# ultralytics/yolov5

Measured on NVIDIA H100. Metric: images/sec @640 (forward + NMS), higher is better.
Workload: dtype bf16

## Files before the change

yolov5_b200/csrc/conv_gemm.cu:

```cuda
#include <cstdio>
#include <cstdlib>
#include <cstring>
#include <mutex>

#include "../../include/y5b200.h"
#include "common.cuh"
#include "host_util.h"
#include "wgmma.cuh"

namespace y5 {

constexpr int kBlockM = 128;
constexpr int kConsumers = 2;
constexpr int kConsumerThreads = 128 * kConsumers;
constexpr int kThreads = 128 + kConsumerThreads;
constexpr int kMaxStages = 8;
constexpr int kHeadN = 128;

enum AMode { A_LINEAR = 0, A_IM2COL = 1, A_PATCH = 2 };

struct ConvParams {
    int M, N;
    int num_m_tiles;
    int num_m_super, num_n_tiles;
    int kh, kw, c_chunks;
    int block_k;
    int a_mode;
    int Ho, Wo, HoWo, stride, pad_h, pad_w;
    int tw, th, tiles_x, tiles_y;
    int b_grouped;
    int patch_pw;
    int cluster_n;
    uint32_t stg_bytes;
    uint32_t b_sub_bytes;
    float rcp_per_img, rcp_tiles_x, rcp_HoWo, rcp_Wo;
    int a_stages, b_stages;
    uint32_t a_sub_bytes, a_stage_bytes, b_stage_bytes;
    int is_bf16, act;
    const float* bias;
    int bias_n;
    void* out;
    int out_pitch;
    const void* res;
    int res_pitch;
    void* raw;
    void* z;
    int na, no, nc, nx, z_rows, z_row0;
    float det_stride;
    float anchor_wh[8];
};

struct SmemLayout {
    uint32_t off_a, off_b, off_out, off_bias, off_bars, total;
};

__host__ __device__ inline SmemLayout smem_layout(int epi, int no, int bias_n, int a_stages, int b_stages, uint32_t a_bytes,
                                                   uint32_t b_bytes, uint32_t stg_bytes) {
    SmemLayout L;
    uint32_t o = 0;
    L.off_a = o;
    o += a_stages * a_bytes;
    L.off_b = o;
    o += b_stages * b_bytes;
    o = (o + 1023) & ~1023u;
    L.off_out = o;
    if (epi == 1) o += 4 * ((kBlockM * no * 2 + 1023) & ~1023u);
    else o += stg_bytes;
    L.off_bias = o;
    o += ((bias_n + 3) & ~3) * 4;
    o = (o + 7) & ~7u;
    L.off_bars = o;
    o += 4 * kMaxStages * 8;
    L.total = o;
    return L;
}

__device__ __forceinline__ int fdiv(int n, int d, float rd) {
    if (n >= (1 << 23)) return n / d;
    int q = __float2int_rz(__int2float_rz(n) * rd);
    const int r = n - q * d;
    if (r >= d) ++q;
    else if (r < 0) --q;
    return q;
}

template <int BLOCK_N, int MT, int KS, bool BF16>
__device__ __forceinline__ void mma_batch(float (&acc)[MT][BLOCK_N / 2], uint32_t a_lo, uint32_t a_sub16, uint32_t a_hi, uint32_t b_lo,
                                          uint32_t b_hi, uint32_t scale_first) {
    wgmma_fence();
#pragma unroll
    for (int k = 0; k < KS; ++k)
#pragma unroll
        for (int mi = 0; mi < MT; ++mi)
            Wgmma<BLOCK_N>::template run<BF16, 0, 0>(acc[mi], gmma_desc(a_lo + mi * a_sub16 + 2 * k, a_hi), gmma_desc(b_lo + 2 * k, b_hi),
                                                     k == 0 ? scale_first : 1u);
    wgmma_commit();
}

template <int BLOCK_N, int EPI, int MT, bool OPT, bool BF16>
__global__ void __launch_bounds__(kThreads, 1)
conv_gemm_kernel(const __grid_constant__ CUtensorMap tmA, const __grid_constant__ CUtensorMap tmB, const ConvParams p) {
    static_assert(MT * BLOCK_N <= 256, "accumulators: at most 128 fp32 registers per consumer thread");
    constexpr int kAcc = BLOCK_N / 2;

    extern __shared__ __align__(1024) uint8_t smem_raw[];
    uint8_t* smem = reinterpret_cast<uint8_t*>((reinterpret_cast<uintptr_t>(smem_raw) + 1023) & ~uintptr_t(1023));
    const SmemLayout L = smem_layout(EPI, p.no, p.bias_n, p.a_stages, p.b_stages, p.a_stage_bytes, p.b_stage_bytes, p.stg_bytes);
    uint8_t* sA = smem + L.off_a;
    uint8_t* sB = smem + L.off_b;
    float* sBias = reinterpret_cast<float*>(smem + L.off_bias);
    uint64_t* a_full = reinterpret_cast<uint64_t*>(smem + L.off_bars);
    uint64_t* a_empty = a_full + kMaxStages;
    uint64_t* b_full = a_empty + kMaxStages;
    uint64_t* b_empty = b_full + kMaxStages;

    const int warp = threadIdx.x >> 5;
    const int lane = threadIdx.x & 31;
    const int csize = OPT ? static_cast<int>(cluster_nctarank()) : 1;
    const uint32_t crank = OPT ? cluster_ctarank() : 0u;

    if (threadIdx.x == 0) {
        tma_prefetch_desc(&tmA);
        tma_prefetch_desc(&tmB);
        for (int s = 0; s < kMaxStages; ++s) {
            mbar_init(&a_full[s], 1);
            mbar_init(&a_empty[s], kConsumers);
            mbar_init(&b_full[s], 1);
            mbar_init(&b_empty[s], kConsumers * csize);
        }
        fence_barrier_init();
    }
    if (threadIdx.x >= 128)
        for (int i = threadIdx.x - 128; i < p.bias_n; i += kConsumerThreads) {
            const float b = i < p.N ? __ldg(p.bias + i) : 0.0f;
            sBias[i] = (EPI == 0 && p.act) ? 0.5f * b : b;
        }
    __syncthreads();
    if (csize > 1) cluster_sync_all();
    griddep_wait();
    griddep_launch_dependents();

    const int nn = p.num_n_tiles;
    const int num_tiles = ((p.num_m_super + csize - 1) / csize) * nn;
    const int tile0 = blockIdx.x / csize, tile_step = gridDim.x / csize;
    const uint32_t row_bytes = p.block_k * 2;
    const bool patch = p.a_mode == A_PATCH;
    const bool wide = OPT && p.patch_pw > 0;
    const int grp = wide ? p.kh * p.kw : (patch ? p.kh : 1);
    const int num_groups = wide ? p.c_chunks : (patch ? p.c_chunks * p.kw : p.kh * p.kw * p.c_chunks);

    if (warp < 4) {
        setmaxnreg_dec<56>();
    }
    if (warp == 0) {
        int as = 0, bs = 0;
        uint32_t aph = 0, bph = 0;
        for (int tile = tile0; tile < num_tiles; tile += tile_step) {
            const int ms = (tile / nn) * csize + static_cast<int>(crank);
            const int n0 = (tile - (tile / nn) * nn) * BLOCK_N;
            int img[MT], y0[MT], x0[MT];
#pragma unroll
            for (int mi = 0; mi < MT; ++mi) {
                const int mt = ms * MT + mi;
                img[mi] = y0[mi] = x0[mi] = 0;
                if (p.a_mode == A_IM2COL) {
                    const int m0 = mt * kBlockM;
                    img[mi] = fdiv(m0, p.HoWo, p.rcp_HoWo);
                    const int rem = m0 - img[mi] * p.HoWo;
                    const int oy = fdiv(rem, p.Wo, p.rcp_Wo);
                    y0[mi] = oy * p.stride - p.pad_h;
                    x0[mi] = (rem - oy * p.Wo) * p.stride - p.pad_w;
                } else if (patch) {
                    const int per_img = p.tiles_x * p.tiles_y;
                    img[mi] = fdiv(mt, per_img, p.rcp_per_img);
                    const int rem = mt - img[mi] * per_img;
                    const int ty = fdiv(rem, p.tiles_x, p.rcp_tiles_x);
                    y0[mi] = ty * p.th - p.pad_h;
                    x0[mi] = (rem - ty * p.tiles_x) * p.tw - p.pad_w;
                }
            }
            auto issue_group = [&](int cc, int s, int r0) {
                mbar_wait(&a_empty[as], aph ^ 1);
                if (elect_one()) {
                    mbar_arrive_expect_tx(&a_full[as], p.a_stage_bytes);
#pragma unroll
                    for (int mi = 0; mi < MT; ++mi) {
                        uint8_t* a_dst = sA + as * p.a_stage_bytes + mi * p.a_sub_bytes;
                        if (wide) {
                            if (mi == 0) tma_load_4d(&tmA, &a_full[as], a_dst, cc * p.block_k, x0[0], y0[0], img[0]);
                        } else if (p.a_mode == A_LINEAR) tma_load_2d(&tmA, &a_full[as], a_dst, cc * p.block_k, (ms * MT + mi) * kBlockM);
                        else if (p.a_mode == A_IM2COL)
                            tma_load_im2col_4d(&tmA, &a_full[as], a_dst, cc * p.block_k, x0[mi], y0[mi], img[mi], static_cast<uint16_t>(s),
                                               static_cast<uint16_t>(r0));
                        else tma_load_4d(&tmA, &a_full[as], a_dst, cc * p.block_k, x0[mi] + s, y0[mi], img[mi]);
                    }
                }
                __syncwarp();
                if (++as == p.a_stages) { as = 0; aph ^= 1; }
// ... 10 lines not shown
                            const int slice_rows = BLOCK_N / csize;
                            tma_load_2d_mcast(&tmB, &b_full[bs], b_dst + crank * slice_rows * row_bytes, kb * p.block_k,
                                              n0 + static_cast<int>(crank) * slice_rows, static_cast<uint16_t>((1u << csize) - 1u));
                        }
                    }
                    __syncwarp();
                    if (stage_last && ++bs == p.b_stages) { bs = 0; bph ^= 1; }
                }
            };
            if (wide) {
                for (int cc = 0; cc < p.c_chunks; ++cc) issue_group(cc, 0, 0);
            } else if (patch) {
                for (int cc = 0; cc < p.c_chunks; ++cc)
                    for (int s = 0; s < p.kw; ++s) issue_group(cc, s, 0);
            } else {
                for (int r = 0; r < p.kh; ++r)
                    for (int s = 0; s < p.kw; ++s)
                        for (int cc = 0; cc < p.c_chunks; ++cc) issue_group(cc, s, r);
            }
        }
    } else if (warp >= 4) {
    setmaxnreg_inc<224>();
    const int wg = (warp >> 2) - 1;
    const int ct = threadIdx.x - 128;
    const int wrow = wg * 64 + (warp & 3) * 16 + (lane >> 2);
    const int ccol = 2 * (lane & 3);
    const bool signal = (threadIdx.x & 127) == 0;
    constexpr bool bf16 = BF16;
    const uint32_t dhi = gmma_desc_hi(row_bytes);
    const uint32_t a_hi = wide ? (dhi & ~0x3FFFu) | (((static_cast<uint32_t>(p.patch_pw) * row_bytes) >> 4) & 0x3FFFu) : dhi;
    const uint32_t a_base = gmma_desc_lo(smem_u32(sA) + (wide ? wg * 8 * p.patch_pw : wg * 64) * row_bytes), b_base = gmma_desc_lo(smem_u32(sB));
    const uint32_t row16 = row_bytes >> 4;
    const uint32_t a_stage16 = p.a_stage_bytes >> 4, b_stage16 = p.b_stage_bytes >> 4, a_sub16 = p.a_sub_bytes >> 4;
    const uint32_t b_sub16 = p.b_sub_bytes >> 4;
    const uint32_t a_shift16 = patch ? (p.tw * row_bytes) >> 4 : 0;
    const int k_steps = p.block_k / 16;
    const int per_img = p.tiles_x * p.tiles_y;
    const int tw_shift = patch ? __ffs(p.tw) - 1 : 0;
    int as = 0, bs = 0, head_set = 0;
    uint32_t aph = 0, bph = 0;
    float acc[MT][kAcc];
#pragma unroll
    for (int mi = 0; mi < MT; ++mi)
#pragma unroll
        for (int i = 0; i < kAcc; ++i) acc[mi][i] = 0.0f;

    int pend_as = 0, pend_bs = 0;
    bool pend_a_last = false, pend_b_last = false;
    auto release_pending = [&]() {
        if (!signal) return;
        if (pend_b_last) {
            if (csize == 1) mbar_arrive(&b_empty[pend_bs]);
            else
                for (int r = 0; r < csize; ++r) mbar_arrive_cluster(mapa_u32(&b_empty[pend_bs], static_cast<uint32_t>(r)));
        }
        if (pend_a_last) mbar_arrive(&a_empty[pend_as]);
    };

    for (int tile = tile0; tile < num_tiles; tile += tile_step) {
        const int ms = (tile / nn) * csize + static_cast<int>(crank);
        const int nt = tile - (tile / nn) * nn;
        const int n0 = nt * BLOCK_N;
        for (int g = 0; g < num_groups; ++g) {
            mbar_wait(&a_full[as], aph);
            const uint32_t a_stage_lo = a_base + as * a_stage16;
            uint32_t a_lo = a_stage_lo;
            for (int j = 0; j < grp; ++j) {
                if (wide) {
                    const int tr = j / p.kw, ts = j - tr * p.kw;
                    a_lo = a_stage_lo + (tr * p.patch_pw + ts) * row16;
                }
                const bool stage_first = !p.b_grouped || j == 0, stage_last = !p.b_grouped || j == grp - 1;
                if (stage_first) mbar_wait(&b_full[bs], bph);
                const uint32_t b_lo = b_base + bs * b_stage16 + (p.b_grouped ? j * b_sub16 : 0u);
                const uint32_t scale_first = (g | j) != 0 ? 1u : 0u;
#pragma unroll
                for (int mi = 0; mi < MT; ++mi) fence_regs(acc[mi]);
                switch (k_steps) {
                    case 4: mma_batch<BLOCK_N, MT, 4, BF16>(acc, a_lo, a_sub16, a_hi, b_lo, dhi, scale_first); break;
                    case 2: mma_batch<BLOCK_N, MT, 2, BF16>(acc, a_lo, a_sub16, a_hi, b_lo, dhi, scale_first); break;
                    default: mma_batch<BLOCK_N, MT, 1, BF16>(acc, a_lo, a_sub16, a_hi, b_lo, dhi, scale_first); break;
                }
                wgmma_wait<1>();
#pragma unroll
                for (int mi = 0; mi < MT; ++mi) fence_regs(acc[mi]);
                if (g | j) release_pending();
                pend_as = as;
                pend_a_last = j == grp - 1;
                pend_bs = bs;
                pend_b_last = stage_last;
                if (stage_last && ++bs == p.b_stages) { bs = 0; bph ^= 1; }
                a_lo += a_shift16;
            }
            if (++as == p.a_stages) { as = 0; aph ^= 1; }
        }
        wgmma_wait<0>();
#pragma unroll
        for (int mi = 0; mi < MT; ++mi) fence_regs(acc[mi]);
        release_pending();

        if (EPI == 0) {
            const bool staged = OPT && p.stg_bytes != 0;
            const uint32_t stg_pitch = BLOCK_N * 2 + 16;
            uint8_t* stg = smem + L.off_out + wg * 64 * stg_pitch;
            auto pixel_of = [&](int mt, int row) -> long long {
                if (patch) {
                    const int img = fdiv(mt, per_img, p.rcp_per_img);
                    const int rem = mt - img * per_img;
                    const int tyi = fdiv(rem, p.tiles_x, p.rcp_tiles_x);
                    const int oy = tyi * p.th + (row >> tw_shift), ox = (rem - tyi * p.tiles_x) * p.tw + (row & ((1 << tw_shift) - 1));
                    return (mt < p.num_m_tiles && oy < p.Ho && ox < p.Wo) ? static_cast<long long>(img) * p.HoWo + oy * p.Wo + ox : -1;
                }
                const long long m = static_cast<long long>(mt) * kBlockM + row;
                return m < p.M ? m : -1;
            };
            constexpr int kRows = 2 * MT, kWords = (OPT ? 128 : 256) / BLOCK_N;
            constexpr int kBatch = kWords < 1 ? 1 : (kWords < kRows ? kWords : kRows);
            const bool has_res = p.res != nullptr;
#pragma unroll
            for (int q0 = 0; q0 < kRows; q0 += kBatch) {
                uint32_t rv[kBatch][BLOCK_N / 8];
                long long gp[kBatch];
#pragma unroll
                for (int q = 0; q < kBatch; ++q) gp[q] = pixel_of(ms * MT + (q0 + q) / 2, wrow + 8 * ((q0 + q) & 1));
                if (has_res) {
#pragma unroll
                    for (int q = 0; q < kBatch; ++q) {
                        const uint16_t* rp = reinterpret_cast<const uint16_t*>(p.res) + (gp[q] < 0 ? 0 : gp[q] * p.res_pitch) + n0 + ccol;
#pragma unroll
                        for (int j = 0; j < BLOCK_N / 8; ++j)
                            rv[q][j] = (gp[q] >= 0 && n0 + 8 * j < p.N) ? *reinterpret_cast<const uint32_t*>(rp + 8 * j) : 0u;
                    }
                }
#pragma unroll
                for (int q = 0; q < kBatch; ++q) {
                    const int mi = (q0 + q) / 2, h = (q0 + q) & 1;
                    const int mt = ms * MT + mi;
                    const int row = wrow + 8 * h;
                    const long long gpix = gp[q];
                    if (gpix >= 0 || staged) {
                        uint16_t* op = reinterpret_cast<uint16_t*>(p.out) + gpix * p.out_pitch + n0 + ccol;
                        uint8_t* sp = stg + (row - wg * 64) * stg_pitch + ccol * 2;
#pragma unroll
                        for (int j = 0; j < BLOCK_N / 8; ++j) {
                            if (n0 + 8 * j >= p.N) continue;
                            const float2 b = *reinterpret_cast<const float2*>(sBias + n0 + 8 * j + ccol);
                            const float a0 = acc[mi][4 * j + 2 * h], a1 = acc[mi][4 * j + 2 * h + 1];
                            float f0, f1;
                            if (p.act) {
                                f0 = silu_from_half(fmaf(a0, 0.5f, b.x));
                                f1 = silu_from_half(fmaf(a1, 0.5f, b.y));
                            } else {
                                f0 = a0 + b.x;
                                f1 = a1 + b.y;
                            }
                            if (has_res && gpix >= 0) {
                                const float2 t = unpack2(rv[q][j], bf16);
                                f0 += t.x;
                                f1 += t.y;
                            }
                            if (staged) *reinterpret_cast<uint32_t*>(sp + 16 * j) = pack2(f0, f1, bf16);
                            else *reinterpret_cast<uint32_t*>(op + 8 * j) = pack2(f0, f1, bf16);
                        }
                    }
                    if (staged && h == 1) {
                        named_bar_sync(2 + wg, 128);
                        constexpr int kSeg = BLOCK_N / 8;
                        for (int i = threadIdx.x & 127; i < 64 * kSeg; i += 128) {
                            const int lrow = i / kSeg, c = i - lrow * kSeg;
                            const long long gp = pixel_of(mt, wg * 64 + lrow);
                            if (gp >= 0 && n0 + 8 * c < p.N)
                                *reinterpret_cast<uint4*>(reinterpret_cast<uint16_t*>(p.out) + gp * p.out_pitch + n0 + 8 * c) =
                                    *reinterpret_cast<const uint4*>(stg + lrow * stg_pitch + c * 16);
                        }
                        named_bar_sync(2 + wg, 128);
                    }
                }
            }
        } else {
            const uint32_t blk = (kBlockM * p.no * 2 + 1023) & ~1023u;
            const int set = head_set;
            head_set ^= 1;
            uint16_t* stage_raw = reinterpret_cast<uint16_t*>(smem + L.off_out + (2 * set) * blk);
            uint16_t* stage_z = reinterpret_cast<uint16_t*>(smem + L.off_out + (2 * set + 1) * blk);
            const int no = p.no;
            const int a = nt;
            const float aw = p.anchor_wh[a * 2], ah = p.anchor_wh[a * 2 + 1];
            const int m0 = ms * kBlockM;
            const int rows_here = min(kBlockM, p.M - m0);
#pragma unroll
            for (int h = 0; h < 2; ++h) {
                const int row = wrow + 8 * h;
                const int m = m0 + row;
                int gx = 0, gy = 0;
                if (m < p.M) { const int pix = m - fdiv(m, p.HoWo, p.rcp_HoWo) * p.HoWo; gy = fdiv(pix, p.nx, p.rcp_Wo); gx = pix - gy * p.nx; }
                const float fgx = static_cast<float>(gx) - 0.5f, fgy = static_cast<float>(gy) - 0.5f;
#pragma unroll
                for (int j = 0; j < BLOCK_N / 8; ++j) {
#pragma unroll
                    for (int e = 0; e < 2; ++e) {
                        const int o = 8 * j + ccol + e;
                        if (o >= no) continue;
                        const float x = acc[0][4 * j + 2 * h + e] + sBias[n0 + o];
                        float d = x;
                        if (o < 5 + p.nc) {
                            const float sg = sigmoid_f(x);
                            if (o == 0) d = (sg * 2.0f + fgx) * p.det_stride;
                            else if (o == 1) d = (sg * 2.0f + fgy) * p.det_stride;
                            else if (o == 2) { const float u = sg * 2.0f; d = u * u * aw; }
                            else if (o == 3) { const float u = sg * 2.0f; d = u * u * ah; }
                            else d = sg;
                        }
                        stage_raw[row * no + o] = pack1(x, bf16);
                        stage_z[row * no + o] = pack1(d, bf16);
                    }
                }
            }
            named_bar_sync(1, kConsumerThreads);
            const int b_lo = fdiv(m0, p.HoWo, p.rcp_HoWo), b_hi = fdiv(m0 + rows_here - 1, p.HoWo, p.rcp_HoWo);
            for (int b = b_lo; b <= b_hi; ++b) {
                const int r_lo = max(b * p.HoWo - m0, 0), r_hi = min((b + 1) * p.HoWo - m0, rows_here);
                const int pix_lo = m0 + r_lo - b * p.HoWo;
                const int n_el = (r_hi - r_lo) * no;
#pragma unroll
                for (int which = 0; which < 2; ++which) {
                    const long long dst_el = which == 0
                        ? ((static_cast<long long>(b) * p.na + a) * p.HoWo + pix_lo) * no
                        : (static_cast<long long>(b) * p.z_rows + p.z_row0 + static_cast<long long>(a) * p.HoWo + pix_lo) * no;
                    uint16_t* dst = reinterpret_cast<uint16_t*>(which == 0 ? p.raw : p.z) + dst_el;
                    const uint16_t* src = (which == 0 ? stage_raw : stage_z) + r_lo * no;
                    if ((((reinterpret_cast<uintptr_t>(dst) | reinterpret_cast<uintptr_t>(src)) & 15) == 0) && (n_el & 7) == 0) {
                        const uint4* s4 = reinterpret_cast<const uint4*>(src);
                        uint4* d4 = reinterpret_cast<uint4*>(dst);
                        for (int i = ct; i < n_el / 8; i += kConsumerThreads) d4[i] = s4[i];
                    } else {
                        for (int i = ct; i < n_el; i += kConsumerThreads) dst[i] = src[i];
                    }
                }
            }
        }
    }
    }
    if (csize > 1) cluster_sync_all();
}

__global__ void conv_direct_kernel(const uint16_t* __restrict__ in, long long xs, long long ys, long long ns, int B, int H,
                                   int W, int Cin, const uint16_t* __restrict__ w, int cin_pad, const float* __restrict__ bias,
                                   uint16_t* out, int out_pitch, int Cout, const uint16_t* res, int res_pitch, int kh, int kw,
                                   int stride, int pad_h, int pad_w, int Ho, int Wo, int act, int bf16) {
    const long long idx = static_cast<long long>(blockIdx.x) * blockDim.x + threadIdx.x;
    const long long total = static_cast<long long>(B) * Ho * Wo * Cout;
    if (idx >= total) return;
    const int n = static_cast<int>(idx % Cout);
    const long long m = idx / Cout;
    const int ox = static_cast<int>(m % Wo);
    const int oy = static_cast<int>((m / Wo) % Ho);
    const int b = static_cast<int>(m / (static_cast<long long>(Wo) * Ho));
    float acc = 0.0f;
    for (int r = 0; r < kh; ++r) {
        const int iy = oy * stride - pad_h + r;
        if (iy < 0 || iy >= H) continue;
        for (int s = 0; s < kw; ++s) {
            const int ix = ox * stride - pad_w + s;
            if (ix < 0 || ix >= W) continue;
            const uint16_t* ip = in + b * ns + iy * ys + ix * xs;
            const uint16_t* wp = w + (static_cast<long long>(n) * kh * kw + r * kw + s) * cin_pad;
            for (int c = 0; c < Cin; ++c) acc += unpack1(ip[c], bf16) * unpack1(wp[c], bf16);
        }
    }
    float x = acc + bias[n];
    if (act) x = x / (1.0f + expf(-x));
    if (res) x += unpack1(res[m * res_pitch + n], bf16);
    out[m * out_pitch + n] = pack1(x, bf16);
}

}

using namespace y5;

namespace {

int pick_block_k(int in_c) {
    return in_c > 16 ? 64 : 16;
}

void pick_tile(int out_c, int64_t m_tiles, int* block_n, int* mt) {
    const int64_t sms = sm_count();
    if (out_c <= 32) { *block_n = 32; *mt = 4; return; }
    if (out_c <= 64) { *block_n = 64; *mt = 2; return; }
    if (out_c <= 128) {
        *block_n = 128;
        *mt = ((m_tiles + 1) / 2) >= sms ? 2 : 1;
        return;
    }
    const int64_t tiles256 = m_tiles * ((out_c + 255) / 256);
    *block_n = (tiles256 >= 2 * sms && (out_c % 256 == 0 || out_c > 384)) ? 256 : 128;
    *mt = 1;
}

int pick_block_n(int out_c, int64_t m_rows) {
    int bn, mt;
    pick_tile(out_c, m_rows > 0 ? (m_rows + kBlockM - 1) / kBlockM : 1, &bn, &mt);
    return bn;
}

template <int BN, int EPI, int MT, bool OPT>
cudaError_t launch_conv(const CUtensorMap& a, const CUtensorMap& b, const ConvParams& p, int grid, int cluster, uint32_t smem,
                        cudaStream_t st) {
    auto* kernel = p.is_bf16 ? conv_gemm_kernel<BN, EPI, MT, OPT, true> : conv_gemm_kernel<BN, EPI, MT, OPT, false>;
    const cudaError_t attr_err = ensure_dyn_smem(reinterpret_cast<const void*>(kernel), 227 * 1024);
    if (attr_err != cudaSuccess) return attr_err;
    count_launch();
    if (cluster == 1) return launch_pdl(kernel, dim3(grid), dim3(kThreads), smem, st, a, b, p);
    static const bool pdl = [] { const char* e = getenv("Y5_PDL"); return !(e && e[0] == '0'); }();
    cudaLaunchConfig_t cfg{};
    cfg.gridDim = dim3(grid);
    cfg.blockDim = dim3(kThreads);
    cfg.dynamicSmemBytes = smem;
    cfg.stream = st;
    cudaLaunchAttribute attr[2];
    attr[0].id = cudaLaunchAttributeClusterDimension;
    attr[0].val.clusterDim.x = cluster;
    attr[0].val.clusterDim.y = 1;
    attr[0].val.clusterDim.z = 1;
    attr[1].id = cudaLaunchAttributeProgrammaticStreamSerialization;
    attr[1].val.programmaticStreamSerializationAllowed = 1;
// ... 13 lines not shown
    ConvParams& p = pc.p;
    p.cluster_n = cluster;
    p.a_stage_bytes = mt * p.a_sub_bytes;
    if (p.patch_pw > 0) p.a_stage_bytes = static_cast<uint32_t>(p.th + p.kh - 1) * p.patch_pw * p.block_k * 2;
    p.num_m_super = (p.num_m_tiles + mt - 1) / mt;
    p.num_n_tiles = epi == 1 ? p.na : (p.N + block_n - 1) / block_n;
    p.bias_n = p.num_n_tiles * block_n;
    const uint32_t budget = 225 * 1024 - 1024;
    const bool patch = p.a_mode == A_PATCH;
    int a_st = 0, b_st = 0;
    if (!patch) {
        for (int s = kMaxStages; s >= 2; --s)
            if (smem_layout(epi, p.no, p.bias_n, s, s, p.a_stage_bytes, p.b_stage_bytes, p.stg_bytes).total <= budget) { a_st = b_st = s; break; }
    } else {
        const int b_min = p.b_grouped ? 2 : 3, b_max = p.b_grouped ? 4 : kMaxStages;
        for (int a = 3; a >= 2 && !a_st; --a)
            for (int b = b_max; b >= b_min; --b)
                if (smem_layout(epi, p.no, p.bias_n, a, b, p.a_stage_bytes, p.b_stage_bytes, p.stg_bytes).total <= budget) { a_st = a; b_st = b; break; }
    }
    if (a_st < 2 || b_st < 2) return set_error(Y5_E_UNSUPPORTED, "conv tile does not fit shared memory (block_n %d a %u b %u)", block_n,
                                                p.a_stage_bytes, p.b_stage_bytes);
    p.a_stages = a_st;
    p.b_stages = b_st;
    pc.smem_bytes = smem_layout(epi, p.no, p.bias_n, a_st, b_st, p.a_stage_bytes, p.b_stage_bytes, p.stg_bytes).total + 1024;
    pc.block_n = block_n;
    pc.epi = epi;
    pc.mt = mt;
    pc.cluster = cluster;
    const long long tiles = static_cast<long long>((p.num_m_super + cluster - 1) / cluster) * p.num_n_tiles;
    const int max_clusters = sm_count() / cluster;
    pc.grid = static_cast<int>(tiles < max_clusters ? tiles : max_clusters) * cluster;
    return 0;
}

int run_plan(const PlanCommon& pc, cudaStream_t st) {
    cudaError_t e = cudaErrorInvalidValue;
    const bool opt = pc.cluster > 1 || pc.p.patch_pw > 0 || pc.p.stg_bytes > 0;
    const int key = (opt ? 100000 : 0) + pc.epi * 10000 + pc.block_n * 10 + pc.mt;
    switch (key) {
        case 324: e = launch_conv<32, 0, 4, false>(pc.tmA, pc.tmB, pc.p, pc.grid, pc.cluster, pc.smem_bytes, st); break;
        case 642: e = launch_conv<64, 0, 2, false>(pc.tmA, pc.tmB, pc.p, pc.grid, pc.cluster, pc.smem_bytes, st); break;
        case 1281: e = launch_conv<128, 0, 1, false>(pc.tmA, pc.tmB, pc.p, pc.grid, pc.cluster, pc.smem_bytes, st); break;
        case 1282: e = launch_conv<128, 0, 2, false>(pc.tmA, pc.tmB, pc.p, pc.grid, pc.cluster, pc.smem_bytes, st); break;
        case 2561: e = launch_conv<256, 0, 1, false>(pc.tmA, pc.tmB, pc.p, pc.grid, pc.cluster, pc.smem_bytes, st); break;
        case 11281: e = launch_conv<kHeadN, 1, 1, false>(pc.tmA, pc.tmB, pc.p, pc.grid, pc.cluster, pc.smem_bytes, st); break;
        case 100324: e = launch_conv<32, 0, 4, true>(pc.tmA, pc.tmB, pc.p, pc.grid, pc.cluster, pc.smem_bytes, st); break;
        case 100642: e = launch_conv<64, 0, 2, true>(pc.tmA, pc.tmB, pc.p, pc.grid, pc.cluster, pc.smem_bytes, st); break;
        case 101281: e = launch_conv<128, 0, 1, true>(pc.tmA, pc.tmB, pc.p, pc.grid, pc.cluster, pc.smem_bytes, st); break;
        case 101282: e = launch_conv<128, 0, 2, true>(pc.tmA, pc.tmB, pc.p, pc.grid, pc.cluster, pc.smem_bytes, st); break;
        case 102561: e = launch_conv<256, 0, 1, true>(pc.tmA, pc.tmB, pc.p, pc.grid, pc.cluster, pc.smem_bytes, st); break;
        default: return set_error(Y5_E_UNSUPPORTED, "conv: no kernel for block_n %d mt %d epi %d", pc.block_n, pc.mt, pc.epi);
    }
    if (e != cudaSuccess) return set_error(int(e), "conv_gemm launch failed: %s", cudaGetErrorString(e));
    return 0;
}

bool aligned16(const void* p) { return (reinterpret_cast<uintptr_t>(p) & 15) == 0; }

struct Geo {
    int kh, kw, pad_h, pad_w, Ho, Wo;
    long long xs, ys, ns;
};
Geo geometry(const y5_conv_desc* d) {
    Geo g;
    g.kh = d->ksize;
    g.kw = d->kw ? d->kw : d->ksize;
    g.pad_h = d->pad;
    g.pad_w = d->kw ? d->pad_w : d->pad;
    g.xs = d->in_x_stride ? d->in_x_stride : d->in_pitch;
    g.ys = d->in_y_stride ? d->in_y_stride : static_cast<long long>(d->in_w) * g.xs;
    g.ns = d->in_n_stride ? d->in_n_stride : static_cast<long long>(d->in_h) * g.ys;
    g.Ho = (d->in_h + 2 * g.pad_h - g.kh) / d->stride + 1;
    g.Wo = (d->in_w + 2 * g.pad_w - g.kw) / d->stride + 1;
    return g;
}

}

struct y5_conv_plan {
    PlanCommon pc;
};
struct y5_detect_plan {
    PlanCommon pc;
};

extern "C" Y5_API int y5_conv_pick(int32_t in_c, int32_t out_c, int64_t m_rows, int32_t* block_k, int32_t* block_n) {
    if (in_c <= 0 || out_c <= 0) return set_error(Y5_E_INVALID, "y5_conv_pick: non-positive channel count");
    if (block_k) *block_k = pick_block_k(in_c);
    if (block_n) *block_n = pick_block_n(out_c, m_rows);
    return 0;
}

static int validate_conv(const y5_conv_desc* d) {
    if (!d || !d->in || !d->weight || !d->bias || !d->out) return set_error(Y5_E_INVALID, "conv: null pointer");
    if (d->dtype != Y5_F16 && d->dtype != Y5_BF16) return set_error(Y5_E_UNSUPPORTED, "conv: dtype must be fp16/bf16");
    if (d->batch <= 0 || d->in_h <= 0 || d->in_w <= 0 || d->in_c <= 0 || d->out_c <= 0)
        return set_error(Y5_E_INVALID, "conv: non-positive dimension");
    const long long xs = d->in_x_stride ? d->in_x_stride : d->in_pitch;
    if (xs <= 0 || xs % 8 || (d->in_y_stride % 8) || (d->in_n_stride % 8) || d->out_pitch < d->out_c || d->out_pitch % 8 || d->out_c % 8)
        return set_error(Y5_E_INVALID, "conv: strides/pitches/out_c must be multiples of 8 elements and cover the view");
    if (!d->in_x_stride && d->in_pitch < d->in_c) return set_error(Y5_E_INVALID, "conv: in_pitch smaller than in_c");
    if (!aligned16(d->in) || !aligned16(d->out) || !aligned16(d->weight) || (d->residual && !aligned16(d->residual)))
        return set_error(Y5_E_INVALID, "conv: pointers must be 16-byte aligned");
    if (d->residual && (d->res_pitch < d->out_c || d->res_pitch % 8)) return set_error(Y5_E_INVALID, "conv: bad residual pitch");
    const int kw = d->kw ? d->kw : d->ksize, pw = d->kw ? d->pad_w : d->pad;
    if (d->ksize < 1 || d->ksize > 7 || kw < 1 || kw > 7 || d->stride < 1 || d->stride > 8 || d->pad < 0 || d->pad > d->ksize || pw < 0 ||
        pw > kw)
        return set_error(Y5_E_UNSUPPORTED, "conv: kernel %dx%d stride %d pad %d,%d unsupported", d->ksize, kw, d->stride, d->pad, pw);
    return 0;
}

extern "C" Y5_API int y5_conv_plan_create(const y5_conv_desc* d, y5_conv_plan** out) {
// ... 6 lines not shown
    if (M64 > 0x7fffffff - 256) return set_error(Y5_E_UNSUPPORTED, "conv: more than 2^31 output pixels");
    const int bk = d->block_k ? d->block_k : pick_block_k(d->in_c);
    if (bk != 16 && bk != 32 && bk != 64) return set_error(Y5_E_INVALID, "conv: block_k must be 16/32/64");
    const bool plain = g.kh == 1 && g.kw == 1 && d->stride == 1 && g.pad_h == 0 && g.pad_w == 0 && !d->in_x_stride && !d->in_y_stride &&
                       !d->in_n_stride;
    int best_tw = 0;
    double best_eff = 0.0;
    if (d->stride == 1 && !plain) {
        for (int tw = 8; tw <= 128; tw <<= 1) {
            const int th = 128 / tw;
            const double eff = (double)g.Wo * g.Ho / ((double)((g.Wo + tw - 1) / tw * tw) * ((g.Ho + th - 1) / th * th));
            if (eff > best_eff + 1e-9) { best_eff = eff; best_tw = tw; }
        }
    }
    int a_mode_sel;
    if (plain) a_mode_sel = A_LINEAR;
    else if (d->a_mode == 2 && d->stride != 1) return set_error(Y5_E_INVALID, "conv: patch mode needs stride 1");
    else if (d->a_mode == 2 || (d->a_mode == 0 && d->stride == 1 && best_eff >= 0.75)) a_mode_sel = A_PATCH;
    else a_mode_sel = A_IM2COL;

    int bn = d->block_n, mt_sel = 0, cl_sel = 1;
    {
        int bn_auto = 0;
        pick_tile(d->out_c, (M64 + kBlockM - 1) / kBlockM, &bn_auto, &mt_sel);
        if (!bn) bn = bn_auto;
        else {
            mt_sel = bn < 128 ? 128 / bn : ((d->reserved & 2) && bn == 128 ? 2 : 1);
            cl_sel = (d->reserved >> 8) > 1 ? (d->reserved >> 8) : 1;
            if (d->reserved & 4) cl_sel = 2;
            if (cl_sel != 1 && cl_sel != 2 && cl_sel != 4) return set_error(Y5_E_INVALID, "conv: cluster size must be 1, 2 or 4");
        }
    }
    if (bn != 32 && bn != 64 && bn != 128 && bn != 256) return set_error(Y5_E_INVALID, "conv: block_n must be 32/64/128/256");
    auto* plan = new y5_conv_plan();
    PlanCommon& pc = plan->pc;
    std::memset(&pc.p, 0, sizeof(pc.p));
    ConvParams& p = pc.p;
    p.M = static_cast<int>(M64);
    p.N = d->out_c;
    p.kh = g.kh; p.kw = g.kw;
    p.Ho = g.Ho; p.Wo = g.Wo; p.HoWo = g.Ho * g.Wo;
    p.rcp_HoWo = 1.0f / static_cast<float>(p.HoWo);
    p.rcp_Wo = 1.0f / static_cast<float>(p.Wo);
    p.stride = d->stride;
    p.pad_h = g.pad_h; p.pad_w = g.pad_w;
    p.is_bf16 = d->dtype == Y5_BF16;
    p.act = d->act;
    p.bias = d->bias;
    p.out = d->out;
    p.out_pitch = d->out_pitch;
// ... 20 lines not shown
        p.a_sub_bytes = kBlockM * row_bytes;
        e = encode_im2col(&pc.tmA, d->dtype, d->in, d->in_c, d->in_w, d->in_h, d->batch, g.xs, g.ys, g.ns, g.kh, g.kw, d->stride, g.pad_h,
                          g.pad_w, bk, kBlockM, sw);
    } else {
        p.tw = best_tw;
        p.th = 128 / best_tw;
        {
            const int tx8 = (g.Wo + 7) / 8, ty16 = (g.Ho + 15) / 16;
            const double eff8 = (double)g.Wo * g.Ho / ((double)tx8 * 8 * ty16 * 16);
            if ((d->reserved & 128) && !(d->reserved & 32) && row_bytes == 128 && g.kw > 1 && (mt_sel == 1 || (mt_sel == 2 && tx8 % 2 == 0)) &&
                eff8 >= best_eff - 1e-9) {
                p.tw = 8;
                p.th = 16;
                p.patch_pw = 8 * mt_sel + 8;
            }
        }
        if (!p.patch_pw && g.kh > 1 && bn <= 128) {
            p.b_grouped = 1;
            p.b_stage_bytes = g.kh * p.b_sub_bytes;
        }
        p.tiles_x = (g.Wo + p.tw - 1) / p.tw;
        p.tiles_y = (g.Ho + p.th - 1) / p.th;
        p.rcp_tiles_x = 1.0f / static_cast<float>(p.tiles_x);
        p.rcp_per_img = 1.0f / static_cast<float>(p.tiles_x * p.tiles_y);
        p.num_m_tiles = d->batch * p.tiles_x * p.tiles_y;
        p.a_sub_bytes = p.patch_pw ? 8 * row_bytes : (p.th + g.kh - 1) * p.tw * row_bytes;
        cuuint64_t dims[4] = {(cuuint64_t)d->in_c, (cuuint64_t)d->in_w, (cuuint64_t)d->in_h, (cuuint64_t)d->batch};
        cuuint64_t str[3] = {(cuuint64_t)g.xs * 2, (cuuint64_t)g.ys * 2, (cuuint64_t)g.ns * 2};
        cuuint32_t box[4] = {(cuuint32_t)bk, (cuuint32_t)(p.patch_pw ? p.patch_pw : p.tw), (cuuint32_t)(p.th + g.kh - 1), 1};
        e = encode_tiled(&pc.tmA, d->dtype, d->in, 4, dims, str, box, sw, "A patch");
    }
    if (e) { delete plan; return e; }
    const uint64_t ktot = static_cast<uint64_t>(p.kh) * p.kw * p.c_chunks * bk;
    {
        cuuint64_t dims[2] = {ktot, (cuuint64_t)d->out_c};
        cuuint64_t str[1] = {ktot * 2};
        cuuint32_t box[2] = {(cuuint32_t)bk, (cuuint32_t)(bn / cl_sel)};
        e = encode_tiled(&pc.tmB, d->dtype, d->weight, 2, dims, str, box, sw, "B");
    }
    if (e) { delete plan; return e; }
    p.stg_bytes = ((d->reserved & 8) && !(d->reserved & 16)) ? static_cast<uint32_t>(kConsumers * 64 * (bn * 2 + 16)) : 0u;
    int e2 = finish_plan(pc, bn, 0, mt_sel, cl_sel);
    if (e2 && p.stg_bytes) {
        p.stg_bytes = 0;
        e2 = finish_plan(pc, bn, 0, mt_sel, cl_sel);
    }
    if (e2) { delete plan; return e2; }
    *out = plan;
    return 0;
}

extern "C" Y5_API int y5_conv_plan_run(const y5_conv_plan* plan, void* stream) {
    if (!plan) return set_error(Y5_E_INVALID, "conv: null plan");
    return run_plan(plan->pc, static_cast<cudaStream_t>(stream));
}
extern "C" Y5_API void y5_conv_plan_destroy(y5_conv_plan* plan) { delete plan; }

extern "C" Y5_API int y5_conv_bn_silu_fwd(const y5_conv_desc* d, void* stream) {
    y5_conv_plan* plan = nullptr;
    if (int e = y5_conv_plan_create(d, &plan)) return e;
    const int e = y5_conv_plan_run(plan, stream);
    y5_conv_plan_destroy(plan);
    return e;
}
// ... 86 lines not shown
```

Measured before the change: 3077.

## Ping-pong consumer warpgroups on alternate tiles to overlap epilogue with MMA

For narrow tiles (MT*BLOCK_N <= 128), each consumer warpgroup now computes a full 128-row tile with doubled accumulators, and the two warpgroups alternate tiles. A turn barrier serializes their mainloops, and stage indices are advanced past the other group's tile. This lets one warpgroup's epilogue overlap the other's MMAs. The change also moves per-tile group counts into params, drops the MT=2 variant for 128-wide tiles, changes the block_n heuristic to use K size and im2col mode, enables staged stores by default for linear non-residual convs, and removes the early griddep_launch_dependents call.

```diff
diff --git a/yolov5_b200/csrc/conv_gemm.cu b/yolov5_b200/csrc/conv_gemm.cu
--- a/yolov5_b200/csrc/conv_gemm.cu
+++ b/yolov5_b200/csrc/conv_gemm.cu
@@ -27,14 +27,18 @@
     int block_k;
     int a_mode;
     int Ho, Wo, HoWo, stride, pad_h, pad_w;
-    int tw, th, tiles_x, tiles_y;
+    int tw, th, tiles_x, tiles_y, per_img;
     int b_grouped;
     int patch_pw;
     int cluster_n;
     uint32_t stg_bytes;
     uint32_t b_sub_bytes;
     float rcp_per_img, rcp_tiles_x, rcp_HoWo, rcp_Wo;
+    int num_tiles;
+    int num_groups, grp;
     int a_stages, b_stages;
+    int a_skip, b_skip;
+    uint32_t a_skip_ph, b_skip_ph;
     uint32_t a_sub_bytes, a_stage_bytes, b_stage_bytes;
     int is_bf16, act;
     const float* bias;
@@ -70,7 +74,7 @@
     o += ((bias_n + 3) & ~3) * 4;
     o = (o + 7) & ~7u;
     L.off_bars = o;
-    o += 4 * kMaxStages * 8;
+    o += (4 * kMaxStages + kConsumers) * 8;
     L.total = o;
     return L;
 }
@@ -84,23 +88,25 @@
     return q;
 }
 
-template <int BLOCK_N, int MT, int KS, bool BF16>
-__device__ __forceinline__ void mma_batch(float (&acc)[MT][BLOCK_N / 2], uint32_t a_lo, uint32_t a_sub16, uint32_t a_hi, uint32_t b_lo,
-                                          uint32_t b_hi, uint32_t scale_first) {
+template <int BLOCK_N, int MT, int H, int KS, bool BF16>
+__device__ __forceinline__ void mma_batch(float (&acc)[H * MT][BLOCK_N / 2], uint32_t a_lo, uint32_t a_sub16, uint32_t a_half16,
+                                          uint32_t a_hi, uint32_t b_lo, uint32_t b_hi, uint32_t scale_first) {
     wgmma_fence();
 #pragma unroll
     for (int k = 0; k < KS; ++k)
 #pragma unroll
-        for (int mi = 0; mi < MT; ++mi)
-            Wgmma<BLOCK_N>::template run<BF16, 0, 0>(acc[mi], gmma_desc(a_lo + mi * a_sub16 + 2 * k, a_hi), gmma_desc(b_lo + 2 * k, b_hi),
-                                                     k == 0 ? scale_first : 1u);
+        for (int u = 0; u < H * MT; ++u)
+            Wgmma<BLOCK_N>::template run<BF16, 0, 0>(acc[u], gmma_desc(a_lo + (u / H) * a_sub16 + (H == 2 ? (u & 1) * a_half16 : 0u) + 2 * k, a_hi),
+                                                     gmma_desc(b_lo + 2 * k, b_hi), k == 0 ? scale_first : 1u);
     wgmma_commit();
 }
 
 template <int BLOCK_N, int EPI, int MT, bool OPT, bool BF16>
 __global__ void __launch_bounds__(kThreads, 1)
 conv_gemm_kernel(const __grid_constant__ CUtensorMap tmA, const __grid_constant__ CUtensorMap tmB, const ConvParams p) {
-    static_assert(MT * BLOCK_N <= 256, "accumulators: at most 128 fp32 registers per consumer thread");
+    constexpr bool kCoop = MT * BLOCK_N > 128;
+    constexpr int kHalves = kCoop ? 1 : 2;
+    static_assert(kHalves * MT * BLOCK_N <= 256, "accumulators: at most 128 fp32 registers per consumer thread");
     constexpr int kAcc = BLOCK_N / 2;
 
     extern __shared__ __align__(1024) uint8_t smem_raw[];
@@ -113,6 +119,7 @@
     uint64_t* a_empty = a_full + kMaxStages;
     uint64_t* b_full = a_empty + kMaxStages;
     uint64_t* b_empty = b_full + kMaxStages;
+    uint64_t* turn = b_empty + kMaxStages;
 
     const int warp = threadIdx.x >> 5;
     const int lane = threadIdx.x & 31;
@@ -124,10 +131,11 @@
         tma_prefetch_desc(&tmB);
         for (int s = 0; s < kMaxStages; ++s) {
             mbar_init(&a_full[s], 1);
-            mbar_init(&a_empty[s], kConsumers);
+            mbar_init(&a_empty[s], kCoop ? kConsumers : 1);
             mbar_init(&b_full[s], 1);
-            mbar_init(&b_empty[s], kConsumers * csize);
-        }
+            mbar_init(&b_empty[s], (kCoop ? kConsumers : 1) * csize);
+        }
+        for (int w = 0; w < kConsumers; ++w) mbar_init(&turn[w], 1);
         fence_barrier_init();
     }
     if (threadIdx.x >= 128)
@@ -138,16 +146,14 @@
     __syncthreads();
     if (csize > 1) cluster_sync_all();
     griddep_wait();
-    griddep_launch_dependents();
 
     const int nn = p.num_n_tiles;
-    const int num_tiles = ((p.num_m_super + csize - 1) / csize) * nn;
+    const int num_tiles = p.num_tiles;
     const int tile0 = blockIdx.x / csize, tile_step = gridDim.x / csize;
     const uint32_t row_bytes = p.block_k * 2;
     const bool patch = p.a_mode == A_PATCH;
     const bool wide = OPT && p.patch_pw > 0;
-    const int grp = wide ? p.kh * p.kw : (patch ? p.kh : 1);
-    const int num_groups = wide ? p.c_chunks : (patch ? p.c_chunks * p.kw : p.kh * p.kw * p.c_chunks);
+    const int grp = p.grp, num_groups = p.num_groups;
 
     if (warp < 4) {
         setmaxnreg_dec<56>();
@@ -171,9 +177,8 @@
                     y0[mi] = oy * p.stride - p.pad_h;
                     x0[mi] = (rem - oy * p.Wo) * p.stride - p.pad_w;
                 } else if (patch) {
-                    const int per_img = p.tiles_x * p.tiles_y;
-                    img[mi] = fdiv(mt, per_img, p.rcp_per_img);
-                    const int rem = mt - img[mi] * per_img;
+                    img[mi] = fdiv(mt, p.per_img, p.rcp_per_img);
+                    const int rem = mt - img[mi] * p.per_img;
                     const int ty = fdiv(rem, p.tiles_x, p.rcp_tiles_x);
                     y0[mi] = ty * p.th - p.pad_h;
                     x0[mi] = (rem - ty * p.tiles_x) * p.tw - p.pad_w;
@@ -230,28 +235,39 @@
     } else if (warp >= 4) {
     setmaxnreg_inc<224>();
     const int wg = (warp >> 2) - 1;
-    const int ct = threadIdx.x - 128;
-    const int wrow = wg * 64 + (warp & 3) * 16 + (lane >> 2);
+    const int wt = threadIdx.x & 127;
+    const int wrow = (warp & 3) * 16 + (lane >> 2);
     const int ccol = 2 * (lane & 3);
-    const bool signal = (threadIdx.x & 127) == 0;
+    const bool signal = wt == 0;
     constexpr bool bf16 = BF16;
     const uint32_t dhi = gmma_desc_hi(row_bytes);
     const uint32_t a_hi = wide ? (dhi & ~0x3FFFu) | (((static_cast<uint32_t>(p.patch_pw) * row_bytes) >> 4) & 0x3FFFu) : dhi;
-    const uint32_t a_base = gmma_desc_lo(smem_u32(sA) + (wide ? wg * 8 * p.patch_pw : wg * 64) * row_bytes), b_base = gmma_desc_lo(smem_u32(sB));
+    const uint32_t a_base = gmma_desc_lo(smem_u32(sA) + (kCoop ? (wide ? wg * 8 * p.patch_pw : wg * 64) * row_bytes : 0u));
+    const uint32_t b_base = gmma_desc_lo(smem_u32(sB));
     const uint32_t row16 = row_bytes >> 4;
+    const uint32_t a_half16 = (wide ? 8 * p.patch_pw : 64) * row16;
     const uint32_t a_stage16 = p.a_stage_bytes >> 4, b_stage16 = p.b_stage_bytes >> 4, a_sub16 = p.a_sub_bytes >> 4;
     const uint32_t b_sub16 = p.b_sub_bytes >> 4;
     const uint32_t a_shift16 = patch ? (p.tw * row_bytes) >> 4 : 0;
     const int k_steps = p.block_k / 16;
-    const int per_img = p.tiles_x * p.tiles_y;
     const int tw_shift = patch ? __ffs(p.tw) - 1 : 0;
-    int as = 0, bs = 0, head_set = 0;
+    int as = 0, bs = 0;
     uint32_t aph = 0, bph = 0;
-    float acc[MT][kAcc];
-#pragma unroll
-    for (int mi = 0; mi < MT; ++mi)
-#pragma unroll
-        for (int i = 0; i < kAcc; ++i) acc[mi][i] = 0.0f;
+    auto skip_tile = [&]() {
+        as += p.a_skip;
+        aph ^= p.a_skip_ph;
+        if (as >= p.a_stages) { as -= p.a_stages; aph ^= 1; }
+        bs += p.b_skip;
+        bph ^= p.b_skip_ph;
+        if (bs >= p.b_stages) { bs -= p.b_stages; bph ^= 1; }
+    };
+    if (!kCoop && wg == 1) skip_tile();
+    uint32_t turn_ph = wg == 0 ? 1u : 0u;
+    float acc[kHalves * MT][kAcc];
+#pragma unroll
+    for (int u = 0; u < kHalves * MT; ++u)
+#pragma unroll
+        for (int i = 0; i < kAcc; ++i) acc[u][i] = 0.0f;
 
     int pend_as = 0, pend_bs = 0;
     bool pend_a_last = false, pend_b_last = false;
@@ -265,10 +281,14 @@
         if (pend_a_last) mbar_arrive(&a_empty[pend_as]);
     };
 
-    for (int tile = tile0; tile < num_tiles; tile += tile_step) {
+    for (int tile = tile0 + (kCoop ? 0 : wg * tile_step); tile < num_tiles; tile += (kCoop ? 1 : kConsumers) * tile_step) {
         const int ms = (tile / nn) * csize + static_cast<int>(crank);
         const int nt = tile - (tile / nn) * nn;
         const int n0 = nt * BLOCK_N;
+        if (!kCoop) {
+            mbar_wait(&turn[wg], turn_ph);
+            turn_ph ^= 1;
+        }
         for (int g = 0; g < num_groups; ++g) {
             mbar_wait(&a_full[as], aph);
             const uint32_t a_stage_lo = a_base + as * a_stage16;
@@ -283,15 +303,15 @@
                 const uint32_t b_lo = b_base + bs * b_stage16 + (p.b_grouped ? j * b_sub16 : 0u);
                 const uint32_t scale_first = (g | j) != 0 ? 1u : 0u;
 #pragma unroll
-                for (int mi = 0; mi < MT; ++mi) fence_regs(acc[mi]);
+                for (int u = 0; u < kHalves * MT; ++u) fence_regs(acc[u]);
                 switch (k_steps) {
-                    case 4: mma_batch<BLOCK_N, MT, 4, BF16>(acc, a_lo, a_sub16, a_hi, b_lo, dhi, scale_first); break;
-                    case 2: mma_batch<BLOCK_N, MT, 2, BF16>(acc, a_lo, a_sub16, a_hi, b_lo, dhi, scale_first); break;
-                    default: mma_batch<BLOCK_N, MT, 1, BF16>(acc, a_lo, a_sub16, a_hi, b_lo, dhi, scale_first); break;
+                    case 4: mma_batch<BLOCK_N, MT, kHalves, 4, BF16>(acc, a_lo, a_sub16, a_half16, a_hi, b_lo, dhi, scale_first); break;
+                    case 2: mma_batch<BLOCK_N, MT, kHalves, 2, BF16>(acc, a_lo, a_sub16, a_half16, a_hi, b_lo, dhi, scale_first); break;
+                    default: mma_batch<BLOCK_N, MT, kHalves, 1, BF16>(acc, a_lo, a_sub16, a_half16, a_hi, b_lo, dhi, scale_first); break;
                 }
                 wgmma_wait<1>();
 #pragma unroll
-                for (int mi = 0; mi < MT; ++mi) fence_regs(acc[mi]);
+                for (int u = 0; u < kHalves * MT; ++u) fence_regs(acc[u]);
                 if (g | j) release_pending();
                 pend_as = as;
                 pend_a_last = j == grp - 1;
@@ -302,10 +322,12 @@
             }
             if (++as == p.a_stages) { as = 0; aph ^= 1; }
         }
+        if (!kCoop && signal) mbar_arrive(&turn[wg ^ 1]);
         wgmma_wait<0>();
 #pragma unroll
-        for (int mi = 0; mi < MT; ++mi) fence_regs(acc[mi]);
+        for (int u = 0; u < kHalves * MT; ++u) fence_regs(acc[u]);
         release_pending();
+        if (!kCoop) skip_tile();
 
         if (EPI == 0) {
             const bool staged = OPT && p.stg_bytes != 0;
@@ -313,8 +335,8 @@
             uint8_t* stg = smem + L.off_out + wg * 64 * stg_pitch;
             auto pixel_of = [&](int mt, int row) -> long long {
                 if (patch) {
-                    const int img = fdiv(mt, per_img, p.rcp_per_img);
-                    const int rem = mt - img * per_img;
+                    const int img = fdiv(mt, p.per_img, p.rcp_per_img);
+                    const int rem = mt - img * p.per_img;
                     const int tyi = fdiv(rem, p.tiles_x, p.rcp_tiles_x);
                     const int oy = tyi * p.th + (row >> tw_shift), ox = (rem - tyi * p.tiles_x) * p.tw + (row & ((1 << tw_shift) - 1));
                     return (mt < p.num_m_tiles && oy < p.Ho && ox < p.Wo) ? static_cast<long long>(img) * p.HoWo + oy * p.Wo + ox : -1;
@@ -322,15 +344,18 @@
                 const long long m = static_cast<long long>(mt) * kBlockM + row;
                 return m < p.M ? m : -1;
             };
-            constexpr int kRows = 2 * MT, kWords = (OPT ? 128 : 256) / BLOCK_N;
-            constexpr int kBatch = kWords < 1 ? 1 : (kWords < kRows ? kWords : kRows);
+            constexpr int kRows = 2 * kHalves * MT, kWords = (OPT ? 128 : 256) / BLOCK_N;
+            constexpr int kMaxRows = OPT ? 2 : 4;
+            constexpr int kBatch = kWords < 1 ? 1 : (kWords < kMaxRows ? kWords : kMaxRows);
             const bool has_res = p.res != nullptr;
+            auto half_of = [&](int u) { return kCoop ? wg : (u & 1); };
+            auto row_of = [&](int q) { return half_of(q >> 1) * 64 + wrow + 8 * (q & 1); };
 #pragma unroll
             for (int q0 = 0; q0 < kRows; q0 += kBatch) {
                 uint32_t rv[kBatch][BLOCK_N / 8];
                 long long gp[kBatch];
 #pragma unroll
-                for (int q = 0; q < kBatch; ++q) gp[q] = pixel_of(ms * MT + (q0 + q) / 2, wrow + 8 * ((q0 + q) & 1));
+                for (int q = 0; q < kBatch; ++q) gp[q] = pixel_of(ms * MT + (q0 + q) / (2 * kHalves), row_of(q0 + q));
                 if (has_res) {
 #pragma unroll
                     for (int q = 0; q < kBatch; ++q) {
@@ -342,18 +367,17 @@
                 }
 #pragma unroll
                 for (int q = 0; q < kBatch; ++q) {
-                    const int mi = (q0 + q) / 2, h = (q0 + q) & 1;
-                    const int mt = ms * MT + mi;
-                    const int row = wrow + 8 * h;
+                    const int u = (q0 + q) / 2, h = (q0 + q) & 1;
+                    const int mt = ms * MT + u / kHalves;
                     const long long gpix = gp[q];
                     if (gpix >= 0 || staged) {
                         uint16_t* op = reinterpret_cast<uint16_t*>(p.out) + gpix * p.out_pitch + n0 + ccol;
-                        uint8_t* sp = stg + (row - wg * 64) * stg_pitch + ccol * 2;
+                        uint8_t* sp = stg + (wrow + 8 * h) * stg_pitch + ccol * 2;
 #pragma unroll
                         for (int j = 0; j < BLOCK_N / 8; ++j) {
                             if (n0 + 8 * j >= p.N) continue;
                             const float2 b = *reinterpret_cast<const float2*>(sBias + n0 + 8 * j + ccol);
-                            const float a0 = acc[mi][4 * j + 2 * h], a1 = acc[mi][4 * j + 2 * h + 1];
+                            const float a0 = acc[u][4 * j + 2 * h], a1 = acc[u][4 * j + 2 * h + 1];
                             float f0, f1;
                             if (p.act) {
                                 f0 = silu_from_half(fmaf(a0, 0.5f, b.x));
@@ -374,9 +398,9 @@
                     if (staged && h == 1) {
                         named_bar_sync(2 + wg, 128);
                         constexpr int kSeg = BLOCK_N / 8;
-                        for (int i = threadIdx.x & 127; i < 64 * kSeg; i += 128) {
+                        for (int i = wt; i < 64 * kSeg; i += 128) {
                             const int lrow = i / kSeg, c = i - lrow * kSeg;
-                            const long long gp = pixel_of(mt, wg * 64 + lrow);
+                            const long long gp = pixel_of(mt, half_of(u) * 64 + lrow);
                             if (gp >= 0 && n0 + 8 * c < p.N)
                                 *reinterpret_cast<uint4*>(reinterpret_cast<uint16_t*>(p.out) + gp * p.out_pitch + n0 + 8 * c) =
                                     *reinterpret_cast<const uint4*>(stg + lrow * stg_pitch + c * 16);
@@ -387,18 +411,17 @@
             }
         } else {
             const uint32_t blk = (kBlockM * p.no * 2 + 1023) & ~1023u;
-            const int set = head_set;
-            head_set ^= 1;
-            uint16_t* stage_raw = reinterpret_cast<uint16_t*>(smem + L.off_out + (2 * set) * blk);
-            uint16_t* stage_z = reinterpret_cast<uint16_t*>(smem + L.off_out + (2 * set + 1) * blk);
+            uint16_t* stage_raw = reinterpret_cast<uint16_t*>(smem + L.off_out + (2 * wg) * blk);
+            uint16_t* stage_z = reinterpret_cast<uint16_t*>(smem + L.off_out + (2 * wg + 1) * blk);
             const int no = p.no;
             const int a = nt;
             const float aw = p.anchor_wh[a * 2], ah = p.anchor_wh[a * 2 + 1];
             const int m0 = ms * kBlockM;
             const int rows_here = min(kBlockM, p.M - m0);
 #pragma unroll
-            for (int h = 0; h < 2; ++h) {
-                const int row = wrow + 8 * h;
+            for (int q = 0; q < 4; ++q) {
+                const int u = q >> 1, h = q & 1;
+                const int row = u * 64 + wrow + 8 * h;
                 const int m = m0 + row;
                 int gx = 0, gy = 0;
                 if (m < p.M) { const int pix = m - fdiv(m, p.HoWo, p.rcp_HoWo) * p.HoWo; gy = fdiv(pix, p.nx, p.rcp_Wo); gx = pix - gy * p.nx; }
@@ -409,7 +432,7 @@
                     for (int e = 0; e < 2; ++e) {
                         const int o = 8 * j + ccol + e;
                         if (o >= no) continue;
-                        const float x = acc[0][4 * j + 2 * h + e] + sBias[n0 + o];
+                        const float x = acc[u][4 * j + 2 * h + e] + sBias[n0 + o];
                         float d = x;
                         if (o < 5 + p.nc) {
                             const float sg = sigmoid_f(x);
@@ -424,7 +447,7 @@
                     }
                 }
             }
-            named_bar_sync(1, kConsumerThreads);
+            named_bar_sync(2 + wg, 128);
             const int b_lo = fdiv(m0, p.HoWo, p.rcp_HoWo), b_hi = fdiv(m0 + rows_here - 1, p.HoWo, p.rcp_HoWo);
             for (int b = b_lo; b <= b_hi; ++b) {
                 const int r_lo = max(b * p.HoWo - m0, 0), r_hi = min((b + 1) * p.HoWo - m0, rows_here);
@@ -440,12 +463,13 @@
                     if ((((reinterpret_cast<uintptr_t>(dst) | reinterpret_cast<uintptr_t>(src)) & 15) == 0) && (n_el & 7) == 0) {
                         const uint4* s4 = reinterpret_cast<const uint4*>(src);
                         uint4* d4 = reinterpret_cast<uint4*>(dst);
-                        for (int i = ct; i < n_el / 8; i += kConsumerThreads) d4[i] = s4[i];
+                        for (int i = wt; i < n_el / 8; i += 128) d4[i] = s4[i];
                     } else {
-                        for (int i = ct; i < n_el; i += kConsumerThreads) dst[i] = src[i];
+                        for (int i = wt; i < n_el; i += 128) dst[i] = src[i];
                     }
                 }
             }
+            named_bar_sync(2 + wg, 128);
         }
     }
     }
@@ -492,24 +516,13 @@
     return in_c > 16 ? 64 : 16;
 }
 
-void pick_tile(int out_c, int64_t m_tiles, int* block_n, int* mt) {
-    const int64_t sms = sm_count();
+void pick_tile(int out_c, int64_t m_tiles, int64_t k_total, bool im2col, int* block_n, int* mt) {
+    *mt = 1;
     if (out_c <= 32) { *block_n = 32; *mt = 4; return; }
     if (out_c <= 64) { *block_n = 64; *mt = 2; return; }
-    if (out_c <= 128) {
-        *block_n = 128;
-        *mt = ((m_tiles + 1) / 2) >= sms ? 2 : 1;
-        return;
-    }
     const int64_t tiles256 = m_tiles * ((out_c + 255) / 256);
-    *block_n = (tiles256 >= 2 * sms && (out_c % 256 == 0 || out_c > 384)) ? 256 : 128;
-    *mt = 1;
-}
-
-int pick_block_n(int out_c, int64_t m_rows) {
-    int bn, mt;
-    pick_tile(out_c, m_rows > 0 ? (m_rows + kBlockM - 1) / kBlockM : 1, &bn, &mt);
-    return bn;
+    const bool wide = out_c >= 256 && (out_c % 256 == 0 || out_c > 384) && tiles256 >= 2 * sm_count();
+    *block_n = wide && (im2col || (k_total >= 2048 && out_c >= 512)) ? 256 : 128;
 }
 
 template <int BN, int EPI, int MT, bool OPT>
@@ -569,12 +582,20 @@
                                                 p.a_stage_bytes, p.b_stage_bytes);
     p.a_stages = a_st;
     p.b_stages = b_st;
+    p.grp = p.patch_pw > 0 ? p.kh * p.kw : (patch ? p.kh : 1);
+    p.num_groups = p.patch_pw > 0 ? p.c_chunks : (patch ? p.c_chunks * p.kw : p.kh * p.kw * p.c_chunks);
+    const int a_per_tile = p.num_groups, b_per_tile = p.b_grouped ? p.num_groups : p.num_groups * p.grp;
+    p.a_skip = a_per_tile % a_st;
+    p.b_skip = b_per_tile % b_st;
+    p.a_skip_ph = (a_per_tile / a_st) & 1;
+    p.b_skip_ph = (b_per_tile / b_st) & 1;
     pc.smem_bytes = smem_layout(epi, p.no, p.bias_n, a_st, b_st, p.a_stage_bytes, p.b_stage_bytes, p.stg_bytes).total + 1024;
     pc.block_n = block_n;
     pc.epi = epi;
     pc.mt = mt;
     pc.cluster = cluster;
     const long long tiles = static_cast<long long>((p.num_m_super + cluster - 1) / cluster) * p.num_n_tiles;
+    p.num_tiles = static_cast<int>(tiles);
     const int max_clusters = sm_count() / cluster;
     pc.grid = static_cast<int>(tiles < max_clusters ? tiles : max_clusters) * cluster;
     return 0;
@@ -588,13 +609,11 @@
         case 324: e = launch_conv<32, 0, 4, false>(pc.tmA, pc.tmB, pc.p, pc.grid, pc.cluster, pc.smem_bytes, st); break;
         case 642: e = launch_conv<64, 0, 2, false>(pc.tmA, pc.tmB, pc.p, pc.grid, pc.cluster, pc.smem_bytes, st); break;
         case 1281: e = launch_conv<128, 0, 1, false>(pc.tmA, pc.tmB, pc.p, pc.grid, pc.cluster, pc.smem_bytes, st); break;
-        case 1282: e = launch_conv<128, 0, 2, false>(pc.tmA, pc.tmB, pc.p, pc.grid, pc.cluster, pc.smem_bytes, st); break;
         case 2561: e = launch_conv<256, 0, 1, false>(pc.tmA, pc.tmB, pc.p, pc.grid, pc.cluster, pc.smem_bytes, st); break;
         case 11281: e = launch_conv<kHeadN, 1, 1, false>(pc.tmA, pc.tmB, pc.p, pc.grid, pc.cluster, pc.smem_bytes, st); break;
         case 100324: e = launch_conv<32, 0, 4, true>(pc.tmA, pc.tmB, pc.p, pc.grid, pc.cluster, pc.smem_bytes, st); break;
         case 100642: e = launch_conv<64, 0, 2, true>(pc.tmA, pc.tmB, pc.p, pc.grid, pc.cluster, pc.smem_bytes, st); break;
         case 101281: e = launch_conv<128, 0, 1, true>(pc.tmA, pc.tmB, pc.p, pc.grid, pc.cluster, pc.smem_bytes, st); break;
-        case 101282: e = launch_conv<128, 0, 2, true>(pc.tmA, pc.tmB, pc.p, pc.grid, pc.cluster, pc.smem_bytes, st); break;
         case 102561: e = launch_conv<256, 0, 1, true>(pc.tmA, pc.tmB, pc.p, pc.grid, pc.cluster, pc.smem_bytes, st); break;
         default: return set_error(Y5_E_UNSUPPORTED, "conv: no kernel for block_n %d mt %d epi %d", pc.block_n, pc.mt, pc.epi);
     }
@@ -634,7 +653,10 @@
 extern "C" Y5_API int y5_conv_pick(int32_t in_c, int32_t out_c, int64_t m_rows, int32_t* block_k, int32_t* block_n) {
     if (in_c <= 0 || out_c <= 0) return set_error(Y5_E_INVALID, "y5_conv_pick: non-positive channel count");
     if (block_k) *block_k = pick_block_k(in_c);
-    if (block_n) *block_n = pick_block_n(out_c, m_rows);
+    if (block_n) {
+        int mt = 1;
+        pick_tile(out_c, m_rows > 0 ? (m_rows + kBlockM - 1) / kBlockM : 1, in_c, false, block_n, &mt);
+    }
     return 0;
 }
 
@@ -687,10 +709,11 @@
     int bn = d->block_n, mt_sel = 0, cl_sel = 1;
     {
         int bn_auto = 0;
-        pick_tile(d->out_c, (M64 + kBlockM - 1) / kBlockM, &bn_auto, &mt_sel);
+        pick_tile(d->out_c, (M64 + kBlockM - 1) / kBlockM, static_cast<int64_t>(g.kh) * g.kw * d->in_c, a_mode_sel == A_IM2COL, &bn_auto,
+                  &mt_sel);
         if (!bn) bn = bn_auto;
         else {
-            mt_sel = bn < 128 ? 128 / bn : ((d->reserved & 2) && bn == 128 ? 2 : 1);
+            mt_sel = bn < 128 ? 128 / bn : 1;
             cl_sel = (d->reserved >> 8) > 1 ? (d->reserved >> 8) : 1;
             if (d->reserved & 4) cl_sel = 2;
             if (cl_sel != 1 && cl_sel != 2 && cl_sel != 4) return set_error(Y5_E_INVALID, "conv: cluster size must be 1, 2 or 4");
@@ -757,8 +780,9 @@
         p.tiles_x = (g.Wo + p.tw - 1) / p.tw;
         p.tiles_y = (g.Ho + p.th - 1) / p.th;
         p.rcp_tiles_x = 1.0f / static_cast<float>(p.tiles_x);
-        p.rcp_per_img = 1.0f / static_cast<float>(p.tiles_x * p.tiles_y);
-        p.num_m_tiles = d->batch * p.tiles_x * p.tiles_y;
+        p.per_img = p.tiles_x * p.tiles_y;
+        p.rcp_per_img = 1.0f / static_cast<float>(p.per_img);
+        p.num_m_tiles = d->batch * p.per_img;
         p.a_sub_bytes = p.patch_pw ? 8 * row_bytes : (p.th + g.kh - 1) * p.tw * row_bytes;
         cuuint64_t dims[4] = {(cuuint64_t)d->in_c, (cuuint64_t)d->in_w, (cuuint64_t)d->in_h, (cuuint64_t)d->batch};
         cuuint64_t str[3] = {(cuuint64_t)g.xs * 2, (cuuint64_t)g.ys * 2, (cuuint64_t)g.ns * 2};
@@ -774,7 +798,8 @@
         e = encode_tiled(&pc.tmB, d->dtype, d->weight, 2, dims, str, box, sw, "B");
     }
     if (e) { delete plan; return e; }
-    p.stg_bytes = ((d->reserved & 8) && !(d->reserved & 16)) ? static_cast<uint32_t>(kConsumers * 64 * (bn * 2 + 16)) : 0u;
+    const bool stage = !(d->reserved & 16) && ((d->reserved & 8) || (p.a_mode == A_LINEAR && !d->residual));
+    p.stg_bytes = stage ? static_cast<uint32_t>(kConsumers * 64 * (bn * 2 + 16)) : 0u;
     int e2 = finish_plan(pc, bn, 0, mt_sel, cl_sel);
     if (e2 && p.stg_bytes) {
         p.stg_bytes = 0;
```

Measured after the change: 3157, median of 6. 2.6% higher.
